# david-wb/tiny-diffusion

Hardware: AMD Instinct MI355X
Metric: train images/s (q_sample+fwd+MSE+bwd+allreduce+Adam), MNIST 28x28 UNet fp32; 1000-step sample latency in `sample` (higher is better)
Workload: dtype f32; 1 GPU; diffusion.py unconditional MNIST 28x28 UNet, fp32, train step, batch 256/GPU (BASELINE.json configs[1]); global_batch=256, per_gpu_batch=256, parallelism=dp1

## Files before the change

### tiny_diffusion_amd/csrc/conv3x3_wino.hip

```cpp
#include "internal.h"
#include "conv_shared.h"

extern unsigned* g_tdx_diag_buffer;
extern size_t g_tdx_diag_bytes;
extern int g_tdx_probe_stamp;

constexpr int WT = 64;
constexpr int WN = 64;
constexpr int WK = 8;
constexpr int A_ST = 16 * WT * WK;
constexpr int B_ST = 16 * WN * WK;
constexpr int STAGE = A_ST + B_ST;

struct WinoArgs {
  const float* in;
  const float* u;
  const float* bias;
  float* out;
  const float* out_scale;
  const float* out_shift;
  float* stats;
  int B, H, W, Cin, Cout, th, tw, NT, tilesN, M;
  float rcp_tpi, rcp_tw;
  int per;
// ... 147 lines not shown
    int rem, tx;
    const int b = div_rcp(T, tpi, a.rcp_tpi, &rem);
    const int ty = div_rcp(rem, a.tw, a.rcp_tw, &tx);
#pragma unroll
    for (int j = 0; j < 4; ++j) {
      const int px = 4 * wave + j;
      const int ih = 2 * ty - 1 + (px >> 2), iw = 2 * tx - 1 + (px & 3);
      const bool ok = tv && (unsigned)ih < (unsigned)a.H && (unsigned)iw < (unsigned)a.W;
      a_off[j][g] = ok ? (unsigned)((((b * a.H + ih) * a.W + iw) * a.Cin + (lane & 1) * 4) * 4) : OOB;
    }
  }
  const unsigned u_base = (unsigned)(nblk * (a.Cin / WK)) * (unsigned)(B_ST * 4) + (unsigned)(wave * 8 * 1024 + lane * 16);

  const int s0 = SPLITK ? (int)blockIdx.y * a.per : 0;
  const int ns = SPLITK ? min(a.per, a.Cin / WK - s0) : a.Cin / WK;
  auto piece = [&](int i, int buf, int k) {
    const int sc = s0 + (k < ns ? k : ns - 1);
    float* Ab = smem + buf * STAGE;
    float* Bb = Ab + A_ST;
    if (i < 8)
      __builtin_amdgcn_raw_ptr_buffer_load_lds(rsrc_u, (lds_ptr_t)(Bb + (wave * 8 + i) * 256), 16, u_base + i * 1024,
                                               (unsigned)sc * (unsigned)(B_ST * 4), 0, 0);
    else
      __builtin_amdgcn_raw_ptr_buffer_load_lds(rsrc_in, (lds_ptr_t)(Ab + (4 * wave + ((i - 8) >> 1)) * 512 + ((i - 8) & 1) * 256), 16,
                                               a_off[(i - 8) >> 1][(i - 8) & 1], (unsigned)(sc * WK * 4), 0, 0);
  };

  constexpr bool PEEL = !SPLITK && EPI != EPI_BNRELU;
  f32x16 acc[16];
  const f32x16 zero16 = {0.f, 0.f, 0.f, 0.f, 0.f, 0.f, 0.f, 0.f, 0.f, 0.f, 0.f, 0.f, 0.f, 0.f, 0.f, 0.f};
  if (!PEEL) {
#pragma unroll
    for (int p = 0; p < 16; ++p)
#pragma unroll
      for (int r = 0; r < 16; ++r) acc[p][r] = 0.f;
  }

#pragma unroll
  for (int i = 0; i < 16; ++i) piece(i, 0, 0);
  unsigned long long t_issued = 0, t_landed = 0, t_loop = 0, c_loop = 0;
  f32x4 d[16], v[16], t1[4], t2[4], t3[4];
  auto xop = [&](int q) {
    const int r = q >> 3, k = q & 7, c = k & 3;
    if (k < 4) {
      if (r == 0) t1[c] = add4(d[4 + c], d[8 + c]);
      else if (r == 1) t2[c] = sub4(d[8 + c], d[4 + c]);
      else t3[c] = sub4(d[4 + c], d[12 + c]);
    } else {
      f32x4(&t)[4] = r == 0 ? t1 : r == 1 ? t2 : t3;
      f32x4& o = v[4 * (r + 1) + c];
      if (c == 0) o = sub4(t[0], t[2]);
      else if (c == 1) o = add4(t[1], t[2]);
      else if (c == 2) o = sub4(t[2], t[1]);
      else o = sub4(t[1], t[3]);
    }
  };
  {
#pragma unroll
    for (int i = 0; i < 8; ++i) piece(i, 1, 1);
    if (a.stamps) t_issued = __builtin_amdgcn_s_memrealtime();
    asm volatile("s_waitcnt vmcnt(8) lgkmcnt(0)\n\ts_barrier" ::: "memory");
    if (a.stamps) { t_landed = __builtin_amdgcn_s_memrealtime(); c_loop = __builtin_amdgcn_s_memtime(); }
    f32x4 bq[5], nbq[2];
    {
      const float* Ab = smem + wm * 256 + l31 * 8 + half * 4;
      const float* Bb = smem + A_ST + wn * 256 + l31 * 8 + half * 4;
#pragma unroll
      for (int c = 0; c < 4; ++c) { d[c] = *reinterpret_cast<const f32x4*>(Ab + c * 512); d[8 + c] = *reinterpret_cast<const f32x4*>(Ab + (8 + c) * 512); }
      nbq[0] = *reinterpret_cast<const f32x4*>(Bb);
      nbq[1] = *reinterpret_cast<const f32x4*>(Bb + 512);
#pragma unroll
      for (int c = 0; c < 4; ++c) { d[4 + c] = *reinterpret_cast<const f32x4*>(Ab + (4 + c) * 512); d[12 + c] = *reinterpret_cast<const f32x4*>(Ab + (12 + c) * 512); }
      f32x4 t0[4];
#pragma unroll
      for (int c = 0; c < 4; ++c) t0[c] = sub4(d[c], d[8 + c]);
      v[0] = sub4(t0[0], t0[2]); v[1] = add4(t0[1], t0[2]); v[2] = sub4(t0[2], t0[1]); v[3] = sub4(t0[1], t0[3]);
    }
    auto stage = [&](auto first_c, int s) {
      constexpr bool FIRST = decltype(first_c)::value;
      const int cb = s & 1;
      const float* Bb = smem + cb * STAGE + A_ST + wn * 256 + l31 * 8 + half * 4;
      const float* An = smem + (cb ^ 1) * STAGE + wm * 256 + l31 * 8 + half * 4;
      const float* Bn = smem + (cb ^ 1) * STAGE + A_ST + wn * 256 + l31 * 8 + half * 4;
      bq[0] = nbq[0]; bq[1] = nbq[1];
      __builtin_amdgcn_sched_barrier(0);
#pragma unroll
      for (int p = 0; p < 16; ++p) {
        const int cur = p % 5;
        if (FIRST) acc[p] = __builtin_amdgcn_mfma_f32_32x32x2f32(v[p][0], bq[cur][0], zero16, 0, 0, 0);
        else acc[p] = __builtin_amdgcn_mfma_f32_32x32x2f32(v[p][0], bq[cur][0], acc[p], 0, 0, 0);
        if (p < 8) piece(8 + p, cb ^ 1, s + 1);
        if (p == 10) bq[4] = *reinterpret_cast<const f32x4*>(Bb + 14 * 512);
        if (p == 11) bq[0] = *reinterpret_cast<const f32x4*>(Bb + 15 * 512);
        if (p == 12) {
          asm volatile("s_waitcnt vmcnt(0) lgkmcnt(0)\n\ts_barrier" ::: "memory");
#pragma unroll
          for (int c = 0; c < 4; ++c) { d[c] = *reinterpret_cast<const f32x4*>(An + c * 512); d[8 + c] = *reinterpret_cast<const f32x4*>(An + (8 + c) * 512); }
        }
        if (p == 13) {
#pragma unroll
          for (int c = 0; c < 4; ++c) d[4 + c] = *reinterpret_cast<const f32x4*>(An + (4 + c) * 512);
        }
        if (p == 14) {
#pragma unroll
          for (int c = 0; c < 4; ++c) t1[c] = sub4(d[c], d[8 + c]);
        }
        if (p == 15) { v[2] = sub4(t1[2], t1[1]); v[3] = sub4(t1[1], t1[3]); }
        __builtin_amdgcn_sched_barrier(0);
        acc[p] = __builtin_amdgcn_mfma_f32_32x32x2f32(v[p][1], bq[cur][1], acc[p], 0, 0, 0);
        if (p < 12) { xop(2 * p); xop(2 * p + 1); }
        else piece(2 * (p - 12), cb, s + 2);
        __builtin_amdgcn_sched_barrier(0);
        acc[p] = __builtin_amdgcn_mfma_f32_32x32x2f32(v[p][2], bq[cur][2], acc[p], 0, 0, 0);
        if (p < 12) bq[(p + 2) % 5] = *reinterpret_cast<const f32x4*>(Bb + (p + 2) * 512);
        if (p == 12) { nbq[0] = *reinterpret_cast<const f32x4*>(Bn); nbq[1] = *reinterpret_cast<const f32x4*>(Bn + 512); }
        if (p == 13) {
#pragma unroll
          for (int c = 0; c < 4; ++c) d[12 + c] = *reinterpret_cast<const f32x4*>(An + (12 + c) * 512);
        }
        if (p == 14) { v[0] = sub4(t1[0], t1[2]); v[1] = add4(t1[1], t1[2]); }
        if (p == 15) piece(7, cb, s + 2);
        __builtin_amdgcn_sched_barrier(0);
        acc[p] = __builtin_amdgcn_mfma_f32_32x32x2f32(v[p][3], bq[cur][3], acc[p], 0, 0, 0);
        if (p >= 12 && p < 15) piece(2 * (p - 12) + 1, cb, s + 2);
        __builtin_amdgcn_sched_barrier(0);
      }
    };
    if (PEEL) stage(std::true_type{}, 0);
    for (int s = PEEL ? 1 : 0; s < ns; ++s) stage(std::false_type{}, s);
    asm volatile("s_waitcnt vmcnt(0) lgkmcnt(0)\n\ts_barrier" ::: "memory");
  }
  if (a.stamps) { t_loop = __builtin_amdgcn_s_memrealtime(); c_loop = __builtin_amdgcn_s_memtime() - c_loop; }
  if (SPLITK)
    wino_epilogue<EPI_PLAIN>(a, a.out + (size_t)blockIdx.y * (size_t)a.M * a.Cout, nullptr, acc, smem, tblk, n0, wm, wn, l31, half, tid);
  else
    wino_epilogue<EPI>(a, a.out, a.bias, acc, smem, tblk, n0, wm, wn, l31, half, tid);
  if (a.stamps && tid == 0) {
    asm volatile("s_waitcnt vmcnt(0)" ::: "memory");
    unsigned long long* o = a.stamps + 8 * ((size_t)blockIdx.y * gridDim.x + blockIdx.x);
    o[0] = t_entry; o[1] = t_issued; o[2] = t_landed; o[3] = t_loop; o[4] = __builtin_amdgcn_s_memrealtime();
    o[5] = c_loop;
    o[6] = __builtin_amdgcn_s_getreg(4 | (0 << 6) | (31 << 11));
    o[7] = __builtin_amdgcn_s_getreg(20 | (0 << 6) | (3 << 11)) & 0xf;
  }
#endif
}

__global__ void __launch_bounds__(512) pack_wino_batch_kernel(TdxWinoPackBatch b) {
  int u = 0;
  while (u + 1 < b.count && (int)blockIdx.x >= b.start[u + 1]) ++u;
  const int cin = b.cin[u], cout = b.cout[u], cin_real = b.cin_real[u];
  const int blk = blockIdx.x - b.start[u];
  const int nkb = cin / 8;
  const int cb = blk / nkb, kb = blk - cb * nkb;
  const int cl = threadIdx.x >> 3, k8 = threadIdx.x & 7;
  const int co = cb * 64 + cl, ci = kb * 8 + k8;
  float g[9];
#pragma unroll
  for (int tap = 0; tap < 9; ++tap) g[tap] = ci < cin_real ? b.w[u][((size_t)co * cin_real + ci) * 9 + tap] : 0.f;
  float gg[4][3], U[16];
#pragma unroll
  for (int c = 0; c < 3; ++c) {
    gg[0][c] = g[c];
    gg[1][c] = 0.5f * (g[c] + g[3 + c] + g[6 + c]);
    gg[2][c] = 0.5f * (g[c] - g[3 + c] + g[6 + c]);
    gg[3][c] = g[6 + c];
  }
#pragma unroll
  for (int r = 0; r < 4; ++r) {
    U[r * 4 + 0] = gg[r][0];
    U[r * 4 + 1] = 0.5f * (gg[r][0] + gg[r][1] + gg[r][2]);
    U[r * 4 + 2] = 0.5f * (gg[r][0] - gg[r][1] + gg[r][2]);
    U[r * 4 + 3] = gg[r][2];
  }
  if (b.uf[u]) {
    float* dst = b.uf[u] + (((size_t)cb * nkb + kb) * 16) * 512 + cl * 8 + k8;
#pragma unroll
    for (int p = 0; p < 16; ++p) dst[p * 512] = U[p];
  }
  if (b.ud[u]) {
    float* dst = b.ud[u] + (((size_t)(ci >> 6) * (cout / 8) + (co >> 3)) * 16) * 512 + (ci & 63) * 8 + (co & 7);
    constexpr int ps = 512;
#pragma unroll
    for (int p = 0; p < 16; ++p) {
      const int xi = p >> 2, nu = p & 3;
      const int sx = xi == 0 ? 3 : xi == 3 ? 0 : xi, sn = nu == 0 ? 3 : nu == 3 ? 0 : nu;
      dst[p * ps] = U[sx * 4 + sn];
    }
  }
}

static int wino_tile_rows(int H, int W) {
  const int th = (H + 1) / 2, tw = (W + 1) / 2;
  if (!(H & 1) && !(W & 1)) return 4 * WT;
  if (WT % (th * tw) == 0) return (WT / (th * tw)) * H * W;
  return 0;
}

extern "C" int tdx_conv3x3_wino_ok(int B, int H, int W, int cin, int cout) {
  if (B <= 0 || H <= 0 || W <= 0 || cin <= 0 || cout <= 0 || cin % WK || cout % WN) return 0;
  if (!wino_tile_rows(H, W)) return 0;
  const int64_t M = (int64_t)B * H * W;
  return M * cin * 4 < (1ll << 31) && M * cout * 4 < (1ll << 31) && (int64_t)cout * 16 * cin * 4 < (1ll << 31) &&
         (int64_t)B * ((H + 1) / 2) * ((W + 1) / 2) + 64 < (1ll << 24);
}

extern "C" int tdx_conv3x3_wino_stat_tile_rows(int B, int H, int W) { (void)B; return wino_tile_rows(H, W); }
extern "C" int tdx_conv3x3_wino_stat_tiles(int B, int H, int W) {
  const int th = (H + 1) / 2, tw = (W + 1) / 2;
  return cdiv((int64_t)B * th * tw, WT);
}

int tdx_pack_conv3x3_wino_pad(const float* w_oihw, float* u_fwd, float* u_dgrad, int cout, int cin_real, int cin,
                              tdx_stream_t stream);

int tdx_pack_conv3x3_wino_batch(TdxWinoPackBatch* b, tdx_stream_t stream) {
  if (!b || b->count <= 0 || b->count > TDX_PACK_MAX) return TDX_E_BADARG;
  int blocks = 0;
  for (int u = 0; u < b->count; ++u) {
    if (!b->w[u] || b->cin_real[u] <= 0 || b->cin_real[u] > b->cin[u] || b->cin[u] % 64 || b->cout[u] % 64) return TDX_E_BADARG;
    b->start[u] = blocks;
    blocks += (b->cin[u] / 8) * (b->cout[u] / 64);
  }
  pack_wino_batch_kernel<<<blocks, 512, 0, to_stream(stream)>>>(*b);
  TDX_CHECK_LAUNCH();
  return 0;
}

int tdx_pack_conv3x3_wino_pad(const float* w_oihw, float* u_fwd, float* u_dgrad, int cout, int cin_real, int cin,
                              tdx_stream_t stream) {
  if (!w_oihw || cout <= 0 || cin <= 0 || cin_real <= 0 || cin_real > cin) return TDX_E_BADARG;
  if (cin % 64 || cout % 64) return TDX_E_SHAPE;
  if (!u_fwd && !u_dgrad) return 0;
  TdxWinoPackBatch b{};
  b.count = 1;
  b.w[0] = w_oihw; b.uf[0] = u_fwd; b.ud[0] = u_dgrad; b.cout[0] = cout; b.cin[0] = cin; b.cin_real[0] = cin_real;
  return tdx_pack_conv3x3_wino_batch(&b, stream);
}

extern "C" int tdx_pack_conv3x3_wino(const float* w_oihw, float* u_fwd, float* u_dgrad, int cout, int cin,
                                     tdx_stream_t stream) {
  return tdx_pack_conv3x3_wino_pad(w_oihw, u_fwd, u_dgrad, cout, cin, cin, stream);
}

int tdx_conv3x3_wino_launch(const float* in, const float* u, const float* bias, float* out, int B, int H, int W,
                            int cin, int cout, int flags, const float* out_scale, const float* out_shift,
                            float* stats_partial, int splits, int per, tdx_stream_t stream) {
  if (!in || !u || !out) return TDX_E_BADARG;
  if (!tdx_conv3x3_wino_ok(B, H, W, cin, cout)) return TDX_E_SHAPE;
  if (flags & ~(TDX_CONV_OUT_BNRELU | TDX_CONV_OUT_STATS)) return TDX_E_BADARG;
  if ((flags & TDX_CONV_OUT_BNRELU) && (!out_scale || !out_shift)) return TDX_E_BADARG;
  if ((flags & TDX_CONV_OUT_STATS) && (!stats_partial || (flags & TDX_CONV_OUT_BNRELU))) return TDX_E_BADARG;
  if (splits < 1 || (splits > 1 && (per < 1 || (int64_t)per * (splits - 1) >= cin / WK))) return TDX_E_BADARG;
  WinoArgs a{};
  a.in = in; a.u = u; a.bias = bias; a.out = out; a.out_scale = out_scale; a.out_shift = out_shift;
  a.stats = stats_partial;
  a.B = B; a.H = H; a.W = W; a.Cin = cin; a.Cout = cout;
  a.th = (H + 1) / 2; a.tw = (W + 1) / 2;
  a.NT = B * a.th * a.tw;
  a.rcp_tpi = 1.0f / (float)(a.th * a.tw); a.rcp_tw = 1.0f / (float)a.tw;
  a.tilesN = cout / WN;
  a.M = B * H * W;
  a.per = per;
  a.compact = cdiv(a.NT, WT) < 64;
  const dim3 grid(a.compact ? cdiv(a.NT, WT) * a.tilesN : (cdiv(a.NT, WT) + 7) / 8 * 8 * a.tilesN, splits);
  a.stamps = g_tdx_probe_stamp == 3 && g_tdx_diag_buffer && (size_t)grid.x * grid.y * 64 <= g_tdx_diag_bytes
                 ? reinterpret_cast<unsigned long long*>(g_tdx_diag_buffer) : nullptr;
  const size_t lds = (size_t)2 * STAGE * sizeof(float) + WT * 2 * sizeof(unsigned);
  hipStream_t st = to_stream(stream);
#define TDX_WINO_LAUNCH(EPI_, SPL_)                                                                              \
  do {                                                                                                           \
    auto kern = conv3x3_wino_kernel<EPI_, SPL_>;                                                                 \
    static bool attr_set = false;                                                                                \
    if (!attr_set) {                                                                                             \
      hipError_t e = hipFuncSetAttribute(reinterpret_cast<const void*>(kern),                                    \
                                         hipFuncAttributeMaxDynamicSharedMemorySize, (int)lds);                  \
      if (e != hipSuccess) return (int)e;                                                                        \
      attr_set = true;                                                                                           \
    }                                                                                                            \
    kern<<<grid, 256, lds, st>>>(a);                                                                             \
  } while (0)
  if (splits > 1) TDX_WINO_LAUNCH(EPI_PLAIN, true);
  else if (flags & TDX_CONV_OUT_BNRELU) TDX_WINO_LAUNCH(EPI_BNRELU, false);
  else if (flags & TDX_CONV_OUT_STATS) TDX_WINO_LAUNCH(EPI_STATS, false);
  else TDX_WINO_LAUNCH(EPI_PLAIN, false);
#undef TDX_WINO_LAUNCH
  TDX_CHECK_LAUNCH();
  return 0;
}

extern "C" int tdx_conv3x3_fwd_wino(const float* in, const float* u, const float* bias, float* out, int B, int H, int W,
                                    int cin, int cout, int flags, const float* out_scale, const float* out_shift,
                                    float* stats_partial, tdx_stream_t stream) {
  return tdx_conv3x3_wino_launch(in, u, bias, out, B, H, W, cin, cout, flags, out_scale, out_shift, stats_partial, 1, 0,
                                 stream);
}

constexpr int GT8 = 8;
constexpr int XS_F = GT8 * 16 * 64;
constexpr int ES_F = GT8 * 4 * 64;
constexpr int WST_F = XS_F + ES_F;
constexpr int WNST = 3;
constexpr int WG_MAX_CHUNK = 1024;

struct WinoWgArgs {
  const float* in;
  const float* dy;
  float* slabs;
  int B, H, W, Cin, Cout, th, tw, NT, M;
  int tilesCo, tilesCi, chunk;
  unsigned long long* stamps;
};

__global__ void __launch_bounds__(256)
conv3x3_wgrad_wino_kernel(WinoWgArgs a) {
#if defined(__HIP_DEVICE_COMPILE__)
  typedef __attribute__((address_space(3))) void* lds_ptr_t;
  typedef int i32x4 __attribute__((ext_vector_type(4)));
  extern __shared__ __attribute__((aligned(16))) float smem[];
  i32x4* tab = reinterpret_cast<i32x4*>(smem + WNST * WST_F);
  const unsigned long long t_entry = a.stamps ? __builtin_amdgcn_s_memrealtime() : 0ull;
  unsigned long long t_table = 0, t_first = 0, t_loop = 0, c_loop = 0;
  const int tid = threadIdx.x;
  const int lane = tid & 63;
  const int wave = __builtin_amdgcn_readfirstlane(tid >> 6);
  const int l31 = lane & 31, half = lane >> 5;
  const int wm = wave >> 1, wn = wave & 1;
  const int ntile = a.tilesCo * a.tilesCi;
  const int split = blockIdx.x / ntile, tl = blockIdx.x - split * ntile;
  const int tile_co = tl / a.tilesCi, tile_ci = tl - tile_co * a.tilesCi;
  const int co0 = tile_co * 64, ci0 = tile_ci * 64;
  const int T_lo = split * a.chunk;
  const int T_hi = min(T_lo + a.chunk, a.NT);
  const int ns = (T_hi - T_lo + GT8 - 1) / GT8;
  const int tpi = a.th * a.tw;
  const int neg = (a.W + 1) * a.Cin;

  for (int i = tid; i < ns * GT8; i += 256) {
    const int T = T_lo + i;
    i32x4 e = {0, 0, 0, 0};
    if (T < T_hi) {
      const int b = T / tpi, rem = T - b * tpi;
      const int ty = rem / a.tw, tx = rem - ty * a.tw;
      e[0] = (((b * a.H + 2 * ty - 1) * a.W + 2 * tx - 1) * a.Cin + neg) * 4;
      e[1] = (((b * a.H + 2 * ty) * a.W + 2 * tx) * a.Cout) * 4;
      int m16 = 0, m4 = 0;
#pragma unroll
      for (int p = 0; p < 16; ++p) {
        const int ih = 2 * ty - 1 + (p >> 2), iw = 2 * tx - 1 + (p & 3);
        if ((unsigned)ih < (unsigned)a.H && (unsigned)iw < (unsigned)a.W) m16 |= 1 << p;
      }
#pragma unroll
      for (int p = 0; p < 4; ++p)
        if (2 * ty + (p >> 1) < a.H && 2 * tx + (p & 1) < a.W) m4 |= 1 << p;
      e[2] = m16; e[3] = m4;
    }
    tab[i] = e;
  }
  __syncthreads();
  if (a.stamps) t_table = __builtin_amdgcn_s_memrealtime();

  const auto rsrc_in = __builtin_amdgcn_make_buffer_rsrc(const_cast<float*>(a.in) - neg, 0,
                                                         (int)(((int64_t)a.M * a.Cin + 2 * neg) * 4), 0x00020000);
  const auto rsrc_dy = __builtin_amdgcn_make_buffer_rsrc(const_cast<float*>(a.dy), 0, (int)((int64_t)a.M * a.Cout * 4), 0x00020000);
  constexpr unsigned OOB = 0x80000000u;
  const int q = lane >> 4, c16 = lane & 15;
  unsigned x_lane[4];
#pragma unroll
  for (int r = 0; r < 4; ++r) x_lane[r] = (unsigned)(((r * a.W + q) * a.Cin + ci0 + c16 * 4) * 4);
  const unsigned dy_lane = (unsigned)((((q >> 1) * a.W + (q & 1)) * a.Cout + co0 + c16 * 4) * 4);

  auto issue_piece = [&](int k, int s, int buf) {
    const int sc = s < ns ? s : ns - 1;
    float* Xb = smem + buf * WST_F;
    float* Eb = Xb + XS_F;
    if (k < 8) {
      const int t = 2 * wave + (k >> 2), r = k & 3;
      const i32x4 e = tab[sc * GT8 + t];
      const bool ok = (e[2] >> (r * 4 + q)) & 1;
      __builtin_amdgcn_raw_ptr_buffer_load_lds(rsrc_in, (lds_ptr_t)(Xb + (t * 16 + r * 4) * 64), 16,
                                               ok ? (unsigned)e[0] + x_lane[r] : OOB, 0, 0, 0);
    } else {
      const int t = 2 * wave + (k - 8);
      const i32x4 e = tab[sc * GT8 + t];
      const bool ok = (e[3] >> q) & 1;
      __builtin_amdgcn_raw_ptr_buffer_load_lds(rsrc_dy, (lds_ptr_t)(Eb + t * 4 * 64), 16, ok ? (unsigned)e[1] + dy_lane : OOB, 0, 0, 0);
    }
  };

  auto issue_piece_e = [&](int k, const i32x4& e0, const i32x4& e1, int buf) {
    float* Xb = smem + buf * WST_F;
    float* Eb = Xb + XS_F;
    if (k < 8) {
      const int t = 2 * wave + (k >> 2), r = k & 3;
      const i32x4& e = (k >> 2) ? e1 : e0;
      const bool ok = (e[2] >> (r * 4 + q)) & 1;
      __builtin_amdgcn_raw_ptr_buffer_load_lds(rsrc_in, (lds_ptr_t)(Xb + (t * 16 + r * 4) * 64), 16,
                                               ok ? (unsigned)e[0] + x_lane[r] : OOB, 0, 0, 0);
    } else {
      const int t = 2 * wave + (k - 8);
      const i32x4& e = (k - 8) ? e1 : e0;
      const bool ok = (e[3] >> q) & 1;
      __builtin_amdgcn_raw_ptr_buffer_load_lds(rsrc_dy, (lds_ptr_t)(Eb + t * 4 * 64), 16, ok ? (unsigned)e[1] + dy_lane : OOB, 0, 0, 0);
    }
  };

  f32x16 acc[16];
#pragma unroll
  for (int p = 0; p < 16; ++p)
#pragma unroll
    for (int r = 0; r < 16; ++r) acc[p][r] = 0.f;

  float Ec[16], Vc[16], En[16], Vn[16];
  float dr[16], er[4];
  const int x_rd = wn * 32 + l31, e_rd = wm * 32 + l31;
  auto read_raw = [&](int buf, int j) {
    const float* Xb = smem + buf * WST_F + (half * 4 + j) * 16 * 64 + x_rd;
    const float* Eb = smem + buf * WST_F + XS_F + (half * 4 + j) * 4 * 64 + e_rd;
#pragma unroll
    for (int p = 0; p < 16; ++p) dr[p] = Xb[p * 64];
#pragma unroll
    for (int p = 0; p < 4; ++p) er[p] = Eb[p * 64];
  };
  float tt[16], aa[4];
  auto xop = [&](int k, float (&V)[16], float (&E)[16]) {
    if (k < 16) {
      const int c = k & 3, w = k >> 2;
      if (w == 0) tt[c] = s_sub(dr[c], dr[8 + c]);
      else if (w == 1) tt[4 + c] = s_add(dr[4 + c], dr[8 + c]);
      else if (w == 2) tt[8 + c] = s_sub(dr[8 + c], dr[4 + c]);
      else tt[12 + c] = s_sub(dr[4 + c], dr[12 + c]);
    } else if (k < 32) {
      const int r = (k - 16) >> 2, w = (k - 16) & 3;
      if (w == 0) V[4 * r] = s_sub(tt[4 * r], tt[4 * r + 2]);
      else if (w == 1) V[4 * r + 1] = s_add(tt[4 * r + 1], tt[4 * r + 2]);
      else if (w == 2) V[4 * r + 2] = s_sub(tt[4 * r + 2], tt[4 * r + 1]);
      else V[4 * r + 3] = s_sub(tt[4 * r + 1], tt[4 * r + 3]);
    } else if (k < 36) {
      const int j = (k - 32) & 1, w = (k - 32) >> 1;
      if (w == 0) aa[j] = s_add(er[j], er[2 + j]);
      else aa[2 + j] = s_sub(er[j], er[2 + j]);
    } else {
      const int xi = (k - 36) >> 1, w = (k - 36) & 1;
      const float a0 = xi == 0 ? er[0] : xi == 1 ? aa[0] : xi == 2 ? aa[2] : er[2];
      const float a1 = xi == 0 ? er[1] : xi == 1 ? aa[1] : xi == 2 ? aa[3] : er[3];
      if (w == 0) { E[4 * xi] = a0; E[4 * xi + 3] = a1; E[4 * xi + 1] = s_add(a0, a1); }
      else E[4 * xi + 2] = s_sub(a0, a1);
    }
  };

#pragma unroll
  for (int k = 0; k < 10; ++k) issue_piece(k, 0, 0);
#pragma unroll
  for (int k = 0; k < 10; ++k) issue_piece(k, 1, 1);
  asm volatile("s_waitcnt vmcnt(10)\n\ts_barrier" ::: "memory");
  read_raw(0, 0);
#pragma unroll
  for (int k = 0; k < 44; ++k) xop(k, Vc, Ec);
  read_raw(0, 1);
  if (a.stamps) { t_first = __builtin_amdgcn_s_memrealtime(); c_loop = __builtin_amdgcn_s_memtime(); }
  float ern[4];
  int b0 = 0;
  for (int s = 0; s < ns; ++s) {
    int b1 = b0 + 1; b1 = b1 == WNST ? 0 : b1;
    int b2 = b1 + 1; b2 = b2 == WNST ? 0 : b2;
    i32x4 e0 = {0, 0, 0, 0}, e1 = {0, 0, 0, 0};
    auto tile_iter = [&](auto Jc) {
      constexpr int J = decltype(Jc)::value;
      if (J == 2) {
        asm volatile("s_waitcnt vmcnt(0) lgkmcnt(0)\n\ts_barrier" ::: "memory");
        const int sc = s + 2 < ns ? s + 2 : ns - 1;
        e0 = tab[sc * GT8 + 2 * wave]; e1 = tab[sc * GT8 + 2 * wave + 1];
      }
      __builtin_amdgcn_sched_barrier(0);
#pragma unroll
      for (int p = 0; p < 16; ++p) {
        acc[p] = __builtin_amdgcn_mfma_f32_32x32x2f32(Ec[p], Vc[p], acc[p], 0, 0, 0);
        if (p & 1) {
#pragma unroll
          for (int k = 0; k < 6; ++k)
            if ((p >> 1) * 6 + k < 44) xop((p >> 1) * 6 + k, Vn, En);
        }
        if (p == 8) {
          const float* Xb = smem + (J < 2 ? b0 : b1) * WST_F + (half * 4 + ((J + 2) & 3)) * 16 * 64 + x_rd;
          const float* Eb = smem + (J < 2 ? b0 : b1) * WST_F + XS_F + (half * 4 + ((J + 2) & 3)) * 4 * 64 + e_rd;
#pragma unroll
          for (int i = 0; i < 16; ++i) dr[i] = Xb[i * 64];
#pragma unroll
          for (int i = 0; i < 4; ++i) ern[i] = Eb[i * 64];
        }
        if ((J == 2 || J == 3) && p % 3 == 1 && p / 3 < 5) issue_piece_e(J == 2 ? p / 3 : 5 + p / 3, e0, e1, b2);
        __builtin_amdgcn_sched_barrier(0);
      }
#pragma unroll
      for (int p = 0; p < 16; ++p) { Ec[p] = En[p]; Vc[p] = Vn[p]; }
#pragma unroll
      for (int i = 0; i < 4; ++i) er[i] = ern[i];
    };
    tile_iter(std::integral_constant<int, 0>{});
    tile_iter(std::integral_constant<int, 1>{});
    tile_iter(std::integral_constant<int, 2>{});
    tile_iter(std::integral_constant<int, 3>{});
    b0 = b1;
  }
  asm volatile("s_waitcnt vmcnt(0) lgkmcnt(0)\n\ts_barrier" ::: "memory");

  if (a.stamps) { t_loop = __builtin_amdgcn_s_memrealtime(); c_loop = __builtin_amdgcn_s_memtime() - c_loop; }

  float* slab = a.slabs + (size_t)split * a.Cout * 9 * a.Cin;
  const int ci = ci0 + wn * 32 + l31;
#pragma unroll
  for (int r = 0; r < 16; ++r) {
    const int co = co0 + wm * 32 + (r & 3) + 8 * (r >> 2) + 4 * half;
    float R[3][4];
#pragma unroll
    for (int nu = 0; nu < 4; ++nu) {
      const float sg = nu == 3 ? -1.f : 1.f;
      const float m0 = sg * acc[0 + nu][r], m1 = sg * acc[4 + nu][r], m2 = sg * acc[8 + nu][r], m3 = -sg * acc[12 + nu][r];
      R[0][nu] = m0 + 0.5f * (m1 + m2);
      R[1][nu] = 0.5f * (m1 - m2);
      R[2][nu] = 0.5f * (m1 + m2) + m3;
    }
#pragma unroll
    for (int k = 0; k < 3; ++k) {
      float* dst = slab + ((size_t)co * 9 + 3 * k) * a.Cin + ci;
      dst[0] = R[k][0] + 0.5f * (R[k][1] + R[k][2]);
      dst[a.Cin] = 0.5f * (R[k][1] - R[k][2]);
      dst[2 * a.Cin] = 0.5f * (R[k][1] + R[k][2]) + R[k][3];
    }
  }
  if (a.stamps && tid == 0) {
    asm volatile("s_waitcnt vmcnt(0)" ::: "memory");
    unsigned long long* o = a.stamps + 8 * (size_t)blockIdx.x;
    o[0] = t_entry; o[1] = t_table; o[2] = t_first; o[3] = t_loop; o[4] = __builtin_amdgcn_s_memrealtime();
    o[5] = c_loop;
    o[6] = __builtin_amdgcn_s_getreg(4 | (0 << 6) | (31 << 11));
    o[7] = __builtin_amdgcn_s_getreg(20 | (0 << 6) | (3 << 11)) & 0xf;
  }
#endif
}

int g_tdx_wino_wgrad_target = 512;
static int wino_wgrad_plan(int NT, int cin, int cout, int* chunk) {
  const int ntile = (cout / 64) * (cin / 64);
  const int target = g_tdx_wino_wgrad_target;
  int splits = (target + ntile - 1) / ntile;
  int ch = (NT + splits - 1) / splits;
  ch = (ch + GT8 - 1) / GT8 * GT8;
  if (ch < 4 * GT8) ch = 4 * GT8;
  if (ch > WG_MAX_CHUNK) ch = WG_MAX_CHUNK;
  *chunk = ch;
  return (NT + ch - 1) / ch;
}

extern "C" int tdx_conv3x3_wgrad_wino_splits(int B, int H, int W, int cin, int cout) {
  if (B <= 0 || H <= 0 || W <= 0 || cin <= 0 || cout <= 0 || cin % 64 || cout % 64) return 0;
  int chunk;
  return wino_wgrad_plan(B * ((H + 1) / 2) * ((W + 1) / 2), cin, cout, &chunk);
}

extern "C" int tdx_conv3x3_wgrad_wino(const float* in, const float* dy, float* dw_slabs, int B, int H, int W, int cin,
                                      int cout, tdx_stream_t stream) {
  if (!in || !dy || !dw_slabs) return TDX_E_BADARG;
  if (B <= 0 || H <= 0 || W <= 0 || cin % 64 || cout % 64 || cin <= 0 || cout <= 0) return TDX_E_SHAPE;
  const int64_t M = (int64_t)B * H * W;
  if ((M * cin + 2 * (int64_t)(W + 1) * cin) * 4 >= (1ll << 31) || M * cout * 4 >= (1ll << 31)) return TDX_E_SHAPE;
  WinoWgArgs a{};
  a.in = in; a.dy = dy; a.slabs = dw_slabs;
  a.B = B; a.H = H; a.W = W; a.Cin = cin; a.Cout = cout;
  a.th = (H + 1) / 2; a.tw = (W + 1) / 2;
  a.NT = B * a.th * a.tw;
  a.M = (int)M;
  a.tilesCo = cout / 64; a.tilesCi = cin / 64;
  const int splits = wino_wgrad_plan(a.NT, cin, cout, &a.chunk);
  const size_t lds = (size_t)WNST * WST_F * sizeof(float) + (size_t)a.chunk * 16;
  static bool attr_set = false;
  if (!attr_set) {
    hipError_t e = hipFuncSetAttribute(reinterpret_cast<const void*>(conv3x3_wgrad_wino_kernel),
                                       hipFuncAttributeMaxDynamicSharedMemorySize,
                                       (int)((size_t)WNST * WST_F * sizeof(float) + (size_t)WG_MAX_CHUNK * 16));
    if (e != hipSuccess) return (int)e;
    attr_set = true;
  }
  a.stamps = g_tdx_probe_stamp == 3 && g_tdx_diag_buffer && (size_t)splits * a.tilesCo * a.tilesCi * 64 <= g_tdx_diag_bytes
                 ? reinterpret_cast<unsigned long long*>(g_tdx_diag_buffer) : nullptr;
  const dim3 grid(splits * a.tilesCo * a.tilesCi);
  conv3x3_wgrad_wino_kernel<<<grid, 256, lds, to_stream(stream)>>>(a);
  TDX_CHECK_LAUNCH();
  return 0;
}
```

Baseline: 25870 images/s.

## Split Winograd wgrad transform across wave pairs and compress tile table

Restructures the Winograd weight-gradient kernel so each pair of waves computes only half of the input-transform rows (H=0/1 templated body). This halves the per-wave transform and LDS read work and the register footprint for V. It also packs the per-tile table into a single 32-bit word with row/column masks, and uses SGPR lane masks with v_cndmask for bounds. The price is an LDS exchange of partial accumulators before the output transform, a fixed 128KB LDS allocation, and more complex code.

```diff
diff --git a/tiny_diffusion_amd/csrc/conv3x3_wino.hip b/tiny_diffusion_amd/csrc/conv3x3_wino.hip
--- a/tiny_diffusion_amd/csrc/conv3x3_wino.hip
+++ b/tiny_diffusion_amd/csrc/conv3x3_wino.hip
@@ -473,6 +473,9 @@
 constexpr int WST_F = XS_F + ES_F;
 constexpr int WNST = 3;
 constexpr int WG_MAX_CHUNK = 1024;
+constexpr int WG_XCH_F = 4 * 8 * 16 * 64;
+constexpr size_t WG_LDS = 131072;
+static_assert((size_t)WNST * WST_F * 4 + (size_t)WG_MAX_CHUNK * 4 <= WG_LDS && (size_t)WG_XCH_F * 4 <= WG_LDS, "LDS");
 
 struct WinoWgArgs {
   const float* in;
@@ -483,20 +486,32 @@
   unsigned long long* stamps;
 };
 
+#if defined(__HIP_DEVICE_COMPILE__)
+__device__ __forceinline__ unsigned long long wg_lanes16(unsigned m) {
+  const unsigned lo = ((m & 1u) ? 0x0000ffffu : 0u) | ((m & 2u) ? 0xffff0000u : 0u);
+  const unsigned hi = ((m & 4u) ? 0x0000ffffu : 0u) | ((m & 8u) ? 0xffff0000u : 0u);
+  return (unsigned long long)hi << 32 | lo;
+}
+__device__ __forceinline__ unsigned wg_sel(unsigned long long mask, unsigned x, unsigned y) {
+  unsigned r;
+  asm("v_cndmask_b32_e64 %0, %1, %2, %3" : "=v"(r) : "v"(y), "v"(x), "s"(mask));
+  return r;
+}
+#endif
+
 __global__ void __launch_bounds__(256)
 conv3x3_wgrad_wino_kernel(WinoWgArgs a) {
 #if defined(__HIP_DEVICE_COMPILE__)
   typedef __attribute__((address_space(3))) void* lds_ptr_t;
-  typedef int i32x4 __attribute__((ext_vector_type(4)));
   extern __shared__ __attribute__((aligned(16))) float smem[];
-  i32x4* tab = reinterpret_cast<i32x4*>(smem + WNST * WST_F);
+  unsigned* tab = reinterpret_cast<unsigned*>(smem + WNST * WST_F);
   const unsigned long long t_entry = a.stamps ? __builtin_amdgcn_s_memrealtime() : 0ull;
   unsigned long long t_table = 0, t_first = 0, t_loop = 0, c_loop = 0;
   const int tid = threadIdx.x;
   const int lane = tid & 63;
   const int wave = __builtin_amdgcn_readfirstlane(tid >> 6);
   const int l31 = lane & 31, half = lane >> 5;
-  const int wm = wave >> 1, wn = wave & 1;
+  const int wn = wave & 1;
   const int ntile = a.tilesCo * a.tilesCi;
   const int split = blockIdx.x / ntile, tl = blockIdx.x - split * ntile;
   const int tile_co = tl / a.tilesCi, tile_ci = tl - tile_co * a.tilesCi;
@@ -509,22 +524,17 @@
 
   for (int i = tid; i < ns * GT8; i += 256) {
     const int T = T_lo + i;
-    i32x4 e = {0, 0, 0, 0};
+    unsigned e = 0;
     if (T < T_hi) {
       const int b = T / tpi, rem = T - b * tpi;
       const int ty = rem / a.tw, tx = rem - ty * a.tw;
-      e[0] = (((b * a.H + 2 * ty - 1) * a.W + 2 * tx - 1) * a.Cin + neg) * 4;
-      e[1] = (((b * a.H + 2 * ty) * a.W + 2 * tx) * a.Cout) * 4;
-      int m16 = 0, m4 = 0;
-#pragma unroll
-      for (int p = 0; p < 16; ++p) {
-        const int ih = 2 * ty - 1 + (p >> 2), iw = 2 * tx - 1 + (p & 3);
-        if ((unsigned)ih < (unsigned)a.H && (unsigned)iw < (unsigned)a.W) m16 |= 1 << p;
+      unsigned rows = 0, cols = 0;
+#pragma unroll
+      for (int p = 0; p < 4; ++p) {
+        if ((unsigned)(2 * ty - 1 + p) < (unsigned)a.H) rows |= 1u << p;
+        if ((unsigned)(2 * tx - 1 + p) < (unsigned)a.W) cols |= 1u << p;
       }
-#pragma unroll
-      for (int p = 0; p < 4; ++p)
-        if (2 * ty + (p >> 1) < a.H && 2 * tx + (p & 1) < a.W) m4 |= 1 << p;
-      e[2] = m16; e[3] = m4;
+      e = (unsigned)((b * a.H + 2 * ty) * a.W + 2 * tx) << 8 | cols << 4 | rows;
     }
     tab[i] = e;
   }
@@ -534,172 +544,212 @@
   const auto rsrc_in = __builtin_amdgcn_make_buffer_rsrc(const_cast<float*>(a.in) - neg, 0,
                                                          (int)(((int64_t)a.M * a.Cin + 2 * neg) * 4), 0x00020000);
   const auto rsrc_dy = __builtin_amdgcn_make_buffer_rsrc(const_cast<float*>(a.dy), 0, (int)((int64_t)a.M * a.Cout * 4), 0x00020000);
-  constexpr unsigned OOB = 0x80000000u;
   const int q = lane >> 4, c16 = lane & 15;
-  unsigned x_lane[4];
-#pragma unroll
-  for (int r = 0; r < 4; ++r) x_lane[r] = (unsigned)(((r * a.W + q) * a.Cin + ci0 + c16 * 4) * 4);
+  const unsigned x_lane = (unsigned)((q * a.Cin + ci0 + c16 * 4) * 4);
   const unsigned dy_lane = (unsigned)((((q >> 1) * a.W + (q & 1)) * a.Cout + co0 + c16 * 4) * 4);
-
-  auto issue_piece = [&](int k, int s, int buf) {
+  const unsigned row_bytes = (unsigned)(a.W * a.Cin * 4), cin4 = (unsigned)a.Cin * 4u, cout4 = (unsigned)a.Cout * 4u;
+  unsigned oob = 0x80000000u;
+  asm volatile("" : "+v"(oob));
+
+  struct Pair { unsigned xb[2], rows[2], db[2]; unsigned long long cm[2], dm[2]; };
+  auto pair_of = [&](uint2 e) {
+    Pair P;
+    const unsigned w[2] = {(unsigned)__builtin_amdgcn_readfirstlane(e.x), (unsigned)__builtin_amdgcn_readfirstlane(e.y)};
+#pragma unroll
+    for (int t = 0; t < 2; ++t) {
+      const unsigned pix = w[t] >> 8, rows = w[t] & 15u, cols = (w[t] >> 4) & 15u;
+      const unsigned r12 = (rows >> 1) & 3u, c12 = (cols >> 1) & 3u;
+      P.xb[t] = pix * cin4;
+      P.rows[t] = rows;
+      P.cm[t] = wg_lanes16(cols);
+      P.db[t] = pix * cout4;
+      P.dm[t] = wg_lanes16(((r12 & 1u) ? c12 : 0u) | ((r12 & 2u) ? c12 << 2 : 0u));
+    }
+    return P;
+  };
+  auto entries = [&](int s) {
     const int sc = s < ns ? s : ns - 1;
+    return *reinterpret_cast<const uint2*>(tab + sc * GT8 + 2 * wave);
+  };
+  auto issue_piece = [&](int k, const Pair& P, int buf) {
     float* Xb = smem + buf * WST_F;
     float* Eb = Xb + XS_F;
     if (k < 8) {
-      const int t = 2 * wave + (k >> 2), r = k & 3;
-      const i32x4 e = tab[sc * GT8 + t];
-      const bool ok = (e[2] >> (r * 4 + q)) & 1;
-      __builtin_amdgcn_raw_ptr_buffer_load_lds(rsrc_in, (lds_ptr_t)(Xb + (t * 16 + r * 4) * 64), 16,
-                                               ok ? (unsigned)e[0] + x_lane[r] : OOB, 0, 0, 0);
+      const int t = k >> 2, r = k & 3;
+      const unsigned long long m = (P.rows[t] >> r) & 1u ? P.cm[t] : 0ull;
+      __builtin_amdgcn_raw_ptr_buffer_load_lds(rsrc_in, (lds_ptr_t)(Xb + ((2 * wave + t) * 16 + r * 4) * 64), 16,
+                                               wg_sel(m, x_lane, oob), P.xb[t] + r * row_bytes, 0, 0);
     } else {
-      const int t = 2 * wave + (k - 8);
-      const i32x4 e = tab[sc * GT8 + t];
-      const bool ok = (e[3] >> q) & 1;
-      __builtin_amdgcn_raw_ptr_buffer_load_lds(rsrc_dy, (lds_ptr_t)(Eb + t * 4 * 64), 16, ok ? (unsigned)e[1] + dy_lane : OOB, 0, 0, 0);
+      const int t = k - 8;
+      __builtin_amdgcn_raw_ptr_buffer_load_lds(rsrc_dy, (lds_ptr_t)(Eb + (2 * wave + t) * 4 * 64), 16,
+                                               wg_sel(P.dm[t], dy_lane, oob), P.db[t], 0, 0);
     }
   };
 
-  auto issue_piece_e = [&](int k, const i32x4& e0, const i32x4& e1, int buf) {
-    float* Xb = smem + buf * WST_F;
-    float* Eb = Xb + XS_F;
-    if (k < 8) {
-      const int t = 2 * wave + (k >> 2), r = k & 3;
-      const i32x4& e = (k >> 2) ? e1 : e0;
-      const bool ok = (e[2] >> (r * 4 + q)) & 1;
-      __builtin_amdgcn_raw_ptr_buffer_load_lds(rsrc_in, (lds_ptr_t)(Xb + (t * 16 + r * 4) * 64), 16,
-                                               ok ? (unsigned)e[0] + x_lane[r] : OOB, 0, 0, 0);
-    } else {
-      const int t = 2 * wave + (k - 8);
-      const i32x4& e = (k - 8) ? e1 : e0;
-      const bool ok = (e[3] >> q) & 1;
-      __builtin_amdgcn_raw_ptr_buffer_load_lds(rsrc_dy, (lds_ptr_t)(Eb + t * 4 * 64), 16, ok ? (unsigned)e[1] + dy_lane : OOB, 0, 0, 0);
+  const int x_rd = wn * 32 + l31;
+  auto body = [&](auto Hc) {
+    constexpr int H = decltype(Hc)::value;
+    f32x16 acc[16];
+#pragma unroll
+    for (int p = 0; p < 16; ++p)
+#pragma unroll
+      for (int r = 0; r < 16; ++r) acc[p][r] = 0.f;
+
+    float Ec[16], Vc[8], En[16], Vn[8];
+    float dr[12], er[8], ern[8];
+    typedef __attribute__((address_space(3))) const float lds_f;
+    typedef float f32x2 __attribute__((ext_vector_type(2)));
+    const unsigned lds0 = (unsigned)(size_t)(lds_f*)smem;
+    const unsigned rx_lane = lds0 + (unsigned)((half * 4 * 16 * 64 + 4 * H * 64 + x_rd) * 4);
+    const unsigned re_lane = lds0 + (unsigned)((XS_F + half * 4 * 4 * 64) * 4 + l31 * 8);
+    auto read_raw = [&](unsigned rx, unsigned re, int j, float (&E)[8]) {
+#pragma unroll
+      for (int p = 0; p < 12; ++p) dr[p] = *(lds_f*)(size_t)(rx + j * 16 * 64 * 4 + p * 256);
+#pragma unroll
+      for (int p = 0; p < 4; ++p) {
+        const f32x2 v = *(const __attribute__((address_space(3))) f32x2*)(size_t)(re + j * 4 * 64 * 4 + p * 256);
+        E[p] = v[0]; E[4 + p] = v[1];
+      }
+    };
+    float tt[8], aa[4];
+    auto xop = [&](int k, float (&V)[8], float (&E)[16]) {
+      if (k < 8) {
+        const int c = k & 3, w = k >> 2;
+        if (H == 0) {
+          if (w == 0) tt[c] = s_sub(dr[c], dr[8 + c]);
+          else tt[4 + c] = s_add(dr[4 + c], dr[8 + c]);
+        } else {
+          if (w == 0) tt[c] = s_sub(dr[4 + c], dr[c]);
+          else tt[4 + c] = s_sub(dr[c], dr[8 + c]);
+        }
+      } else if (k < 16) {
+        const int r = (k - 8) >> 2, w = (k - 8) & 3;
+        if (w == 0) V[4 * r] = s_sub(tt[4 * r], tt[4 * r + 2]);
+        else if (w == 1) V[4 * r + 1] = s_add(tt[4 * r + 1], tt[4 * r + 2]);
+        else if (w == 2) V[4 * r + 2] = s_sub(tt[4 * r + 2], tt[4 * r + 1]);
+        else V[4 * r + 3] = s_sub(tt[4 * r + 1], tt[4 * r + 3]);
+      } else {
+        const int c2 = (k - 16) / 6, w = (k - 16) % 6;
+        const float* e = er + 4 * c2;
+        float* a2 = aa + 2 * c2;
+        if (w < 2) a2[w] = H == 0 ? s_add(e[w], e[2 + w]) : s_sub(e[w], e[2 + w]);
+        else {
+          const int x = (w - 2) >> 1;
+          const float a0 = (H == 0) == (x == 0) ? e[2 * H] : a2[0];
+          const float a1 = (H == 0) == (x == 0) ? e[2 * H + 1] : a2[1];
+          float* o = E + 8 * c2 + 4 * x;
+          if ((w & 1) == 0) { o[0] = a0; o[3] = a1; o[1] = s_add(a0, a1); }
+          else o[2] = s_sub(a0, a1);
+        }
+      }
+    };
+
+    {
+      const Pair P0 = pair_of(entries(0));
+#pragma unroll
+      for (int k = 0; k < 10; ++k) issue_piece(k, P0, 0);
+      const Pair P1 = pair_of(entries(1));
+#pragma unroll
+      for (int k = 0; k < 10; ++k) issue_piece(k, P1, 1);
+    }
+    asm volatile("s_waitcnt vmcnt(10)\n\ts_barrier" ::: "memory");
+    read_raw(rx_lane, re_lane, 0, er);
+#pragma unroll
+    for (int k = 0; k < 28; ++k) xop(k, Vc, Ec);
+    read_raw(rx_lane, re_lane, 1, er);
+    if (a.stamps) { t_first = __builtin_amdgcn_s_memrealtime(); c_loop = __builtin_amdgcn_s_memtime(); }
+    unsigned rx0 = rx_lane, re0 = re_lane;
+    int b0 = 0;
+    for (int s = 0; s < ns; ++s) {
+      int b1 = b0 + 1; b1 = b1 == WNST ? 0 : b1;
+      int b2 = b1 + 1; b2 = b2 == WNST ? 0 : b2;
+      unsigned rx1 = rx_lane + (unsigned)(b1 * WST_F * 4), re1 = re_lane + (unsigned)(b1 * WST_F * 4);
+      asm volatile("" : "+v"(rx1), "+v"(re1));
+      uint2 e2 = {0u, 0u};
+      Pair P;
+      auto tile_iter = [&](auto Jc) {
+        constexpr int J = decltype(Jc)::value;
+        if (J == 2) {
+          asm volatile("s_waitcnt vmcnt(0) lgkmcnt(0)\n\ts_barrier" ::: "memory");
+          e2 = entries(s + 2);
+        }
+        __builtin_amdgcn_sched_barrier(0);
+#pragma unroll
+        for (int p = 0; p < 16; ++p) {
+          acc[p] = __builtin_amdgcn_mfma_f32_32x32x2f32(Ec[p], Vc[p & 7], acc[p], 0, 0, 0);
+          if (p & 1) {
+#pragma unroll
+            for (int k = 0; k < 4; ++k)
+              if ((p >> 1) * 4 + k < 28) xop((p >> 1) * 4 + k, Vn, En);
+          }
+          if (p == 8) read_raw(J < 2 ? rx0 : rx1, J < 2 ? re0 : re1, (J + 2) & 3, ern);
+          if (J == 2 && p == 1) P = pair_of(e2);
+          if ((J == 2 || J == 3) && p % 3 == 1 && p / 3 < 5) issue_piece(J == 2 ? p / 3 : 5 + p / 3, P, b2);
+          __builtin_amdgcn_sched_barrier(0);
+        }
+#pragma unroll
+        for (int p = 0; p < 16; ++p) Ec[p] = En[p];
+#pragma unroll
+        for (int p = 0; p < 8; ++p) { Vc[p] = Vn[p]; er[p] = ern[p]; }
+      };
+      tile_iter(std::integral_constant<int, 0>{});
+      tile_iter(std::integral_constant<int, 1>{});
+      tile_iter(std::integral_constant<int, 2>{});
+      tile_iter(std::integral_constant<int, 3>{});
+      b0 = b1; rx0 = rx1; re0 = re1;
+    }
+    asm volatile("s_waitcnt vmcnt(0) lgkmcnt(0)\n\ts_barrier" ::: "memory");
+
+    if (a.stamps) { t_loop = __builtin_amdgcn_s_memrealtime(); c_loop = __builtin_amdgcn_s_memtime() - c_loop; }
+
+    {
+      f32x4* xo = reinterpret_cast<f32x4*>(smem) + ((1 - H) * 2 + wn) * 2048 + lane;
+#pragma unroll
+      for (int p = 0; p < 8; ++p)
+#pragma unroll
+        for (int r4 = 0; r4 < 4; ++r4) {
+          const f32x16& v = acc[8 * (1 - H) + p];
+          xo[(p * 4 + r4) * 64] = f32x4{v[4 * r4], v[4 * r4 + 1], v[4 * r4 + 2], v[4 * r4 + 3]};
+        }
+    }
+    __syncthreads();
+    float* slab = a.slabs + (size_t)split * a.Cout * 9 * a.Cin;
+    const int ci = ci0 + wn * 32 + l31;
+    const f32x4* xin = reinterpret_cast<const f32x4*>(smem) + wave * 2048 + lane;
+#pragma unroll
+    for (int r4 = 0; r4 < 4; ++r4) {
+      f32x4 pv[8];
+#pragma unroll
+      for (int p = 0; p < 8; ++p) pv[p] = xin[(p * 4 + r4) * 64];
+#pragma unroll
+      for (int rr = 0; rr < 4; ++rr) {
+        const int r = 4 * r4 + rr;
+        const int co = co0 + 2 * ((r & 3) + 8 * (r >> 2) + 4 * half) + H;
+        auto M = [&](int x, int nu) {
+          return (x >> 1) == H ? acc[8 * H + 4 * (x & 1) + nu][r] : pv[4 * (x & 1) + nu][rr];
+        };
+        float R[3][4];
+#pragma unroll
+        for (int nu = 0; nu < 4; ++nu) {
+          const float sg = nu == 3 ? -1.f : 1.f;
+          const float m0 = sg * M(0, nu), m1 = sg * M(1, nu), m2 = sg * M(2, nu), m3 = -sg * M(3, nu);
+          R[0][nu] = m0 + 0.5f * (m1 + m2);
+          R[1][nu] = 0.5f * (m1 - m2);
+          R[2][nu] = 0.5f * (m1 + m2) + m3;
+        }
+#pragma unroll
+        for (int k = 0; k < 3; ++k) {
+          float* dst = slab + ((size_t)co * 9 + 3 * k) * a.Cin + ci;
+          dst[0] = R[k][0] + 0.5f * (R[k][1] + R[k][2]);
+          dst[a.Cin] = 0.5f * (R[k][1] - R[k][2]);
+          dst[2 * a.Cin] = 0.5f * (R[k][1] + R[k][2]) + R[k][3];
+        }
+      }
     }
   };
-
-  f32x16 acc[16];
-#pragma unroll
-  for (int p = 0; p < 16; ++p)
-#pragma unroll
-    for (int r = 0; r < 16; ++r) acc[p][r] = 0.f;
-
-  float Ec[16], Vc[16], En[16], Vn[16];
-  float dr[16], er[4];
-  const int x_rd = wn * 32 + l31, e_rd = wm * 32 + l31;
-  auto read_raw = [&](int buf, int j) {
-    const float* Xb = smem + buf * WST_F + (half * 4 + j) * 16 * 64 + x_rd;
-    const float* Eb = smem + buf * WST_F + XS_F + (half * 4 + j) * 4 * 64 + e_rd;
-#pragma unroll
-    for (int p = 0; p < 16; ++p) dr[p] = Xb[p * 64];
-#pragma unroll
-    for (int p = 0; p < 4; ++p) er[p] = Eb[p * 64];
-  };
-  float tt[16], aa[4];
-  auto xop = [&](int k, float (&V)[16], float (&E)[16]) {
-    if (k < 16) {
-      const int c = k & 3, w = k >> 2;
-      if (w == 0) tt[c] = s_sub(dr[c], dr[8 + c]);
-      else if (w == 1) tt[4 + c] = s_add(dr[4 + c], dr[8 + c]);
-      else if (w == 2) tt[8 + c] = s_sub(dr[8 + c], dr[4 + c]);
-      else tt[12 + c] = s_sub(dr[4 + c], dr[12 + c]);
-    } else if (k < 32) {
-      const int r = (k - 16) >> 2, w = (k - 16) & 3;
-      if (w == 0) V[4 * r] = s_sub(tt[4 * r], tt[4 * r + 2]);
-      else if (w == 1) V[4 * r + 1] = s_add(tt[4 * r + 1], tt[4 * r + 2]);
-      else if (w == 2) V[4 * r + 2] = s_sub(tt[4 * r + 2], tt[4 * r + 1]);
-      else V[4 * r + 3] = s_sub(tt[4 * r + 1], tt[4 * r + 3]);
-    } else if (k < 36) {
-      const int j = (k - 32) & 1, w = (k - 32) >> 1;
-      if (w == 0) aa[j] = s_add(er[j], er[2 + j]);
-      else aa[2 + j] = s_sub(er[j], er[2 + j]);
-    } else {
-      const int xi = (k - 36) >> 1, w = (k - 36) & 1;
-      const float a0 = xi == 0 ? er[0] : xi == 1 ? aa[0] : xi == 2 ? aa[2] : er[2];
-      const float a1 = xi == 0 ? er[1] : xi == 1 ? aa[1] : xi == 2 ? aa[3] : er[3];
-      if (w == 0) { E[4 * xi] = a0; E[4 * xi + 3] = a1; E[4 * xi + 1] = s_add(a0, a1); }
-      else E[4 * xi + 2] = s_sub(a0, a1);
-    }
-  };
-
-#pragma unroll
-  for (int k = 0; k < 10; ++k) issue_piece(k, 0, 0);
-#pragma unroll
-  for (int k = 0; k < 10; ++k) issue_piece(k, 1, 1);
-  asm volatile("s_waitcnt vmcnt(10)\n\ts_barrier" ::: "memory");
-  read_raw(0, 0);
-#pragma unroll
-  for (int k = 0; k < 44; ++k) xop(k, Vc, Ec);
-  read_raw(0, 1);
-  if (a.stamps) { t_first = __builtin_amdgcn_s_memrealtime(); c_loop = __builtin_amdgcn_s_memtime(); }
-  float ern[4];
-  int b0 = 0;
-  for (int s = 0; s < ns; ++s) {
-    int b1 = b0 + 1; b1 = b1 == WNST ? 0 : b1;
-    int b2 = b1 + 1; b2 = b2 == WNST ? 0 : b2;
-    i32x4 e0 = {0, 0, 0, 0}, e1 = {0, 0, 0, 0};
-    auto tile_iter = [&](auto Jc) {
-      constexpr int J = decltype(Jc)::value;
-      if (J == 2) {
-        asm volatile("s_waitcnt vmcnt(0) lgkmcnt(0)\n\ts_barrier" ::: "memory");
-        const int sc = s + 2 < ns ? s + 2 : ns - 1;
-        e0 = tab[sc * GT8 + 2 * wave]; e1 = tab[sc * GT8 + 2 * wave + 1];
-      }
-      __builtin_amdgcn_sched_barrier(0);
-#pragma unroll
-      for (int p = 0; p < 16; ++p) {
-        acc[p] = __builtin_amdgcn_mfma_f32_32x32x2f32(Ec[p], Vc[p], acc[p], 0, 0, 0);
-        if (p & 1) {
-#pragma unroll
-          for (int k = 0; k < 6; ++k)
-            if ((p >> 1) * 6 + k < 44) xop((p >> 1) * 6 + k, Vn, En);
-        }
-        if (p == 8) {
-          const float* Xb = smem + (J < 2 ? b0 : b1) * WST_F + (half * 4 + ((J + 2) & 3)) * 16 * 64 + x_rd;
-          const float* Eb = smem + (J < 2 ? b0 : b1) * WST_F + XS_F + (half * 4 + ((J + 2) & 3)) * 4 * 64 + e_rd;
-#pragma unroll
-          for (int i = 0; i < 16; ++i) dr[i] = Xb[i * 64];
-#pragma unroll
-          for (int i = 0; i < 4; ++i) ern[i] = Eb[i * 64];
-        }
-        if ((J == 2 || J == 3) && p % 3 == 1 && p / 3 < 5) issue_piece_e(J == 2 ? p / 3 : 5 + p / 3, e0, e1, b2);
-        __builtin_amdgcn_sched_barrier(0);
-      }
-#pragma unroll
-      for (int p = 0; p < 16; ++p) { Ec[p] = En[p]; Vc[p] = Vn[p]; }
-#pragma unroll
-      for (int i = 0; i < 4; ++i) er[i] = ern[i];
-    };
-    tile_iter(std::integral_constant<int, 0>{});
-    tile_iter(std::integral_constant<int, 1>{});
-    tile_iter(std::integral_constant<int, 2>{});
-    tile_iter(std::integral_constant<int, 3>{});
-    b0 = b1;
-  }
-  asm volatile("s_waitcnt vmcnt(0) lgkmcnt(0)\n\ts_barrier" ::: "memory");
-
-  if (a.stamps) { t_loop = __builtin_amdgcn_s_memrealtime(); c_loop = __builtin_amdgcn_s_memtime() - c_loop; }
-
-  float* slab = a.slabs + (size_t)split * a.Cout * 9 * a.Cin;
-  const int ci = ci0 + wn * 32 + l31;
-#pragma unroll
-  for (int r = 0; r < 16; ++r) {
-    const int co = co0 + wm * 32 + (r & 3) + 8 * (r >> 2) + 4 * half;
-    float R[3][4];
-#pragma unroll
-    for (int nu = 0; nu < 4; ++nu) {
-      const float sg = nu == 3 ? -1.f : 1.f;
-      const float m0 = sg * acc[0 + nu][r], m1 = sg * acc[4 + nu][r], m2 = sg * acc[8 + nu][r], m3 = -sg * acc[12 + nu][r];
-      R[0][nu] = m0 + 0.5f * (m1 + m2);
-      R[1][nu] = 0.5f * (m1 - m2);
-      R[2][nu] = 0.5f * (m1 + m2) + m3;
-    }
-#pragma unroll
-    for (int k = 0; k < 3; ++k) {
-      float* dst = slab + ((size_t)co * 9 + 3 * k) * a.Cin + ci;
-      dst[0] = R[k][0] + 0.5f * (R[k][1] + R[k][2]);
-      dst[a.Cin] = 0.5f * (R[k][1] - R[k][2]);
-      dst[2 * a.Cin] = 0.5f * (R[k][1] + R[k][2]) + R[k][3];
-    }
-  }
+  if (wave >> 1) body(std::integral_constant<int, 1>{});
+  else body(std::integral_constant<int, 0>{});
+
   if (a.stamps && tid == 0) {
     asm volatile("s_waitcnt vmcnt(0)" ::: "memory");
     unsigned long long* o = a.stamps + 8 * (size_t)blockIdx.x;
@@ -744,19 +794,17 @@
   a.M = (int)M;
   a.tilesCo = cout / 64; a.tilesCi = cin / 64;
   const int splits = wino_wgrad_plan(a.NT, cin, cout, &a.chunk);
-  const size_t lds = (size_t)WNST * WST_F * sizeof(float) + (size_t)a.chunk * 16;
   static bool attr_set = false;
   if (!attr_set) {
     hipError_t e = hipFuncSetAttribute(reinterpret_cast<const void*>(conv3x3_wgrad_wino_kernel),
-                                       hipFuncAttributeMaxDynamicSharedMemorySize,
-                                       (int)((size_t)WNST * WST_F * sizeof(float) + (size_t)WG_MAX_CHUNK * 16));
+                                       hipFuncAttributeMaxDynamicSharedMemorySize, (int)WG_LDS);
     if (e != hipSuccess) return (int)e;
     attr_set = true;
   }
   a.stamps = g_tdx_probe_stamp == 3 && g_tdx_diag_buffer && (size_t)splits * a.tilesCo * a.tilesCi * 64 <= g_tdx_diag_bytes
                  ? reinterpret_cast<unsigned long long*>(g_tdx_diag_buffer) : nullptr;
   const dim3 grid(splits * a.tilesCo * a.tilesCi);
-  conv3x3_wgrad_wino_kernel<<<grid, 256, lds, to_stream(stream)>>>(a);
+  conv3x3_wgrad_wino_kernel<<<grid, 256, WG_LDS, to_stream(stream)>>>(a);
   TDX_CHECK_LAUNCH();
   return 0;
 }
```

New measurement: 26440 images/s (median of 6 runs). 1.02x the previous value.
